# GrumpyZhou/patch2pix

Measured on AMD Instinct MI355X. Metric: image-pairs/sec (480x640, ptmax=400), matching hot path, feature pyramids resident in HBM, higher is better.
Workload: dtype f32-equivalent: fp16x2 (every f32 operand, scaled by an exact power of two, = sum of 2 fp16 planes to within 2^-24 of its magnitude; 3 fp16 MFMA products per f32 product, f32 accumulate); second convolution as Winograd F(2x2,3x3) (transforms in f32, filters transformed in f64)

## Files before the change

patch2pix_amd/csrc/regress_wino.hip:

```cpp
#ifndef WNPL
#define WNPL 2
#endif
#include "regress_common.h"

#include <algorithm>
#include <cmath>
#include <vector>

#undef WNS
#if WNPL == 1
#define WNS(f) fp16x1::f
#else
#define WNS(f) f
#endif

namespace p2p {
#if WNPL == 1
namespace fp16x1 {
#endif

typedef _Float16 we8 __attribute__((ext_vector_type(8)));
#define WMFMA(a, b, c) __builtin_amdgcn_mfma_f32_32x32x16_f16(__builtin_bit_cast(we8, (a)), __builtin_bit_cast(we8, (b)), (c), 0, 0, 0)

constexpr int WNT = 512;
constexpr int WBLK = WNPL * (WINO_BLK / 2);
constexpr int WPIECE = WBLK / 8;
constexpr int WSTAGE = 2 * WBLK;
constexpr int WRING = 4;
constexpr int WLDS = WRING * WSTAGE;
static_assert(WINO_BLK == 2 * 128 * 64, "block = [plane 2][row 128][32 K of fp16]");

struct WinoArgs {
    const unsigned char *U;
    const unsigned char *Wt;
    const float *bn2s, *bn2b;
    const float *hinv;
    float *V;
    int mblocks;
    int p0, n;
    const int *dev_counts;
    int nitems;
    int start[MAXB + 1];
};

#if WNPL == 2
#define WDMA(ga_, gb_, la_)                                                                                            \
        P2P_GLOBAL_LOAD_LDS16(ga_ + lane16, la_, 0); P2P_GLOBAL_LOAD_LDS16(ga_ + lane16, la_, 1024);                   \
        P2P_GLOBAL_LOAD_LDS16(gb_ + lane16, la_ + WBLK, 0); P2P_GLOBAL_LOAD_LDS16(gb_ + lane16, la_ + WBLK, 1024);
#define WWAIT_TWO_IN_FLIGHT() P2P_WAIT_VMCNT(8)
#define WWAIT_ONE_IN_FLIGHT() P2P_WAIT_VMCNT(4)
#else
#undef WDMA
#undef WWAIT_TWO_IN_FLIGHT
#undef WWAIT_ONE_IN_FLIGHT
#define WDMA(ga_, gb_, la_)                                                                                            \
        P2P_GLOBAL_LOAD_LDS16(ga_ + lane16, la_, 0); P2P_GLOBAL_LOAD_LDS16(gb_ + lane16, la_ + WBLK, 0);
#define WWAIT_TWO_IN_FLIGHT() P2P_WAIT_VMCNT(4)
#define WWAIT_ONE_IN_FLIGHT() P2P_WAIT_VMCNT(2)
#endif
#define WISSUE(ST, SLOT)                                                                                               \
    {                                                                                                                  \
        const int st_ = (ST) < 256 ? (ST) : 255;            \
        const int p_ = st_ >> 4, kc_ = st_ & 15;                                                                       \
        const unsigned char *ga_ = a.U + ((size_t)(p_ * a.mblocks + mb) * 16 + kc_) * WBLK + woff;                      \
        const unsigned char *gb_ = a.Wt + ((size_t)((p_ * 4 + nb) * 16 + kc_)) * WBLK + woff;                           \
        unsigned char *la_ = smb + (SLOT) * WSTAGE + wave * WPIECE;                                                    \
        WDMA(ga_, gb_, la_)                                                                                            \
    }
#define WREAD(FA, FB, SLOT, S)                                                                                         \
    {                                                                                                                  \
        const unsigned char *pa_ = smb + (SLOT) * WSTAGE + ((S) ? aoff1 : aoff0);                                      \
        const unsigned char *pb_ = smb + (SLOT) * WSTAGE + WBLK + ((S) ? boff1 : boff0);                                \
        _Pragma("unroll") for (int q_ = 0; q_ < WNPL; ++q_) {                                                           \
            FA[0][q_] = *(const f32x4 *)(pa_ + q_ * 8192);                                                             \
            FA[1][q_] = *(const f32x4 *)(pa_ + 2048 + q_ * 8192);                                                      \
            FB[q_] = *(const f32x4 *)(pb_ + q_ * 8192);                                                                \
        }                                                                                                              \
    }
#if WNPL == 2
#define WSLAB_(FA, FB, C0, C1)                                                                                         \
    M0 = WMFMA(FA[0][1], FB[0], C0); M1 = WMFMA(FA[1][1], FB[0], C1);                                                  \
    M0 = WMFMA(FA[0][0], FB[1], M0); M1 = WMFMA(FA[1][0], FB[1], M1);                                                  \
    M0 = WMFMA(FA[0][0], FB[0], M0); M1 = WMFMA(FA[1][0], FB[0], M1);
#else
#undef WSLAB_
#define WSLAB_(FA, FB, C0, C1) M0 = WMFMA(FA[0][0], FB[0], C0); M1 = WMFMA(FA[1][0], FB[0], C1);
#endif
#define WSLAB(FA, FB) WSLAB_(FA, FB, M0, M1)
#define WSLABZ(FA, FB) WSLAB_(FA, FB, zero16, zero16)

#if WNPL == 2
#define WPIPE_A()                                                                                                      \
    _Pragma("unroll") for (int g_ = 0; g_ < 6; ++g_) {                                                                 \
        __builtin_amdgcn_sched_group_barrier(0x008, 1, 0); __builtin_amdgcn_sched_group_barrier(0x100, 1, 0); }        \
    __builtin_amdgcn_sched_barrier(0);
#define WPIPE_B()                                                                                                      \
    _Pragma("unroll") for (int g_ = 0; g_ < 4; ++g_) {                                                                 \
        __builtin_amdgcn_sched_group_barrier(0x008, 1, 0); __builtin_amdgcn_sched_group_barrier(0x010, 1, 0);          \
        __builtin_amdgcn_sched_group_barrier(0x100, 1, 0); }                                                           \
    _Pragma("unroll") for (int g_ = 0; g_ < 2; ++g_) {                                                                 \
        __builtin_amdgcn_sched_group_barrier(0x008, 1, 0); __builtin_amdgcn_sched_group_barrier(0x100, 1, 0); }        \
    __builtin_amdgcn_sched_barrier(0);
#else
#undef WPIPE_A
#undef WPIPE_B
#define WPIPE_A()                                                                                                      \
    __builtin_amdgcn_sched_group_barrier(0x008, 1, 0); __builtin_amdgcn_sched_group_barrier(0x100, 2, 0);              \
    __builtin_amdgcn_sched_group_barrier(0x008, 1, 0); __builtin_amdgcn_sched_group_barrier(0x100, 1, 0);              \
    __builtin_amdgcn_sched_barrier(0);
#define WPIPE_B()                                                                                                      \
    __builtin_amdgcn_sched_group_barrier(0x008, 1, 0); __builtin_amdgcn_sched_group_barrier(0x010, 1, 0);              \
    __builtin_amdgcn_sched_group_barrier(0x100, 2, 0);                                                                 \
    __builtin_amdgcn_sched_group_barrier(0x008, 1, 0); __builtin_amdgcn_sched_group_barrier(0x010, 1, 0);              \
    __builtin_amdgcn_sched_group_barrier(0x100, 1, 0);                                                                 \
    __builtin_amdgcn_sched_barrier(0);
#endif

__global__ __launch_bounds__(WNT, 1) void wino_gemm_kernel(WinoArgs a) {
    P2P_DYN_SHARED(unsigned char, smb);
    const int tid = threadIdx.x;
    const int wave = __builtin_amdgcn_readfirstlane(tid >> 6);
    const int lane = tid & 63, l31 = lane & 31, half = lane >> 5;
    const int g = blockIdx.x, xcd = g & 7, q = g >> 3;
    const int nb = q & 3, mb = (q >> 2) * 8 + xcd;
    if (mb >= a.mblocks || wino_slot(a, a.p0 + mb * 8) < 0) return;
    const int wm = wave >> 2, wn = wave & 3;
    const unsigned lane16 = lane * 16, woff = wave * WPIECE;
    const int sw = (l31 >> 2) & 3;
    const unsigned aoff0 = ((wm * 64 + l31) * 4 + ((0 + half) ^ sw)) * 16, aoff1 = ((wm * 64 + l31) * 4 + ((2 + half) ^ sw)) * 16;
    const unsigned boff0 = ((wn * 32 + l31) * 4 + ((0 + half) ^ sw)) * 16, boff1 = ((wn * 32 + l31) * 4 + ((2 + half) ^ sw)) * 16;

    const f32x16 zero16 = {0};
    f32x16 Y[4][2];
#pragma unroll
    for (int ab = 0; ab < 4; ++ab)
#pragma unroll
        for (int t = 0; t < 2; ++t) Y[ab][t] = zero16;
    f32x4 XA[2][WNPL], XB[WNPL], YA[2][WNPL], YB[WNPL];

    WISSUE(0, 0) WISSUE(1, 1) WISSUE(2, 2)
    WWAIT_TWO_IN_FLIGHT();
    __builtin_amdgcn_s_barrier();
    WREAD(XA, XB, 0, 0)
    __builtin_amdgcn_sched_barrier(0);

#pragma unroll 1
    for (int p = 0; p < 16; ++p) {
        f32x16 M0, M1;
#pragma unroll
        for (int kc = 0; kc < 16; ++kc) {
            const int slot = kc & 3;
            WREAD(YA, YB, slot, 1)
            if (kc == 0) { WSLABZ(XA, XB) } else { WSLAB(XA, XB) }
            WPIPE_A()
            WWAIT_ONE_IN_FLIGHT();
            __builtin_amdgcn_s_barrier();
            __builtin_amdgcn_sched_barrier(0);
            WISSUE(p * 16 + kc + 3, (kc + 3) & 3)
            WREAD(XA, XB, (kc + 1) & 3, 0)
            WSLAB(YA, YB)
            WPIPE_B()
        }
        {
            const int i = p >> 2, j = p & 3;
            const float ca[2] = {(i < 3) ? 1.f : 0.f, (i == 0) ? 0.f : (i == 1) ? 1.f : -1.f};
            const float cb[2] = {(j < 3) ? 1.f : 0.f, (j == 0) ? 0.f : (j == 1) ? 1.f : -1.f};
#pragma unroll
            for (int ab = 0; ab < 4; ++ab) {
                const float c = ca[ab >> 1] * cb[ab & 1];
                Y[ab][0] += c * M0; Y[ab][1] += c * M1;
            }
        }
    }
    P2P_WAIT_VMCNT(0);

    const int n = nb * 128 + wn * 32 + l31;
    const float s = a.bn2s[n], b = a.bn2b[n];
#pragma unroll
    for (int t = 0; t < 2; ++t)
#pragma unroll
        for (int gq = 0; gq < 2; ++gq) {
            const int pl = mb * 8 + wm * 4 + 2 * t + gq;
            const int slot = wino_slot(a, a.p0 + pl);
            const float hs = s * a.hinv[pl];
            float m = 0.f;
#pragma unroll
            for (int ab = 0; ab < 4; ++ab)
#pragma unroll
                for (int r = 0; r < 8; ++r) m = fmaxf(m, fmaf(Y[ab][t][8 * gq + r], hs, b));
            m = fmaxf(m, __shfl_xor(m, 32));
            if (half == 0 && slot >= 0) a.V[(size_t)slot * 512 + n] = m;
        }
}

__global__ __launch_bounds__(WNT) void wino_zero_tail_kernel(WinoArgs a, unsigned char *U, float *hinv, int p1) {
    const int mb = blockIdx.x, tid = threadIdx.x, wave = tid >> 6, lane = tid & 63;
    if (wino_slot(a, a.p0 + mb * 8) < 0) return;
    for (int j = 1; j < 8; ++j) {
        const int c = a.p0 + mb * 8 + j;
        if (c < p1 && wino_slot(a, c) >= 0) continue;
        const unsigned rr = (unsigned)j * 16u + ((unsigned)lane >> 2);
        const unsigned inblk = (rr * 4u + (((unsigned)lane & 3u) ^ ((rr >> 2) & 3u))) * 16u;
        const size_t pstride = (size_t)a.mblocks * (16u * WBLK);
        for (int i2 = 0; i2 < 2; ++i2) {
            unsigned char *ub = U + (size_t)(((unsigned)mb * 16u + (unsigned)(wave * 2 + i2)) * (unsigned)WBLK + inblk);
            for (int pos = 0; pos < 16; ++pos) {
                *(uint4 *)(ub + pos * pstride) = make_uint4(0u, 0u, 0u, 0u);
#if WNPL == 2
                *(uint4 *)(ub + pos * pstride + WINO_BLK / 2) = make_uint4(0u, 0u, 0u, 0u);
#endif
            }
        }
        if (tid == 0) hinv[mb * 8 + j] = 0.f;
    }
}

#if WNPL == 2
__global__ __launch_bounds__(NT, 2) void regress_fc_kernel(RegressArgs args, int lvl) {
    P2P_DYN_SHARED(unsigned char, smb);
    fc_batch_parse(args.reg[lvl], args, lvl, args.ws + (size_t)lvl * args.n * 512,
                   args.ws + ((2 * (size_t)args.n * 512 + 31) & ~(size_t)31), smb, threadIdx.x);
}
#endif

void pack_wino_weights(const float *conv2_w, float *out, int *t2) {
    static const double G[4][3] = {{1, 0, 0}, {0.5, 0.5, 0.5}, {0.5, -0.5, 0.5}, {0, 0, 1}};
    std::vector<double> wt((size_t)16 * 512 * 512);
    std::vector<double> mx(512, 0.0);
    for (int n = 0; n < 512; ++n)
        for (int k = 0; k < 512; ++k) {
            const float *gk = conv2_w + ((size_t)n * 512 + k) * 9;
            double tmp[4][3];
            for (int i = 0; i < 4; ++i)
                for (int b = 0; b < 3; ++b) tmp[i][b] = G[i][0] * gk[0 * 3 + b] + G[i][1] * gk[1 * 3 + b] + G[i][2] * gk[2 * 3 + b];
            for (int i = 0; i < 4; ++i)
                for (int j = 0; j < 4; ++j) {
                    const double v = tmp[i][0] * G[j][0] + tmp[i][1] * G[j][1] + tmp[i][2] * G[j][2];
                    wt[((size_t)(i * 4 + j) * 512 + n) * 512 + k] = v;
                    mx[n] = std::max(mx[n], std::fabs(v));
                }
        }
    for (int n = 0; n < 512; ++n) t2[n] = plane_exponent(mx[n]);
    uint16_t *d = (uint16_t *)out;
    for (int p = 0; p < 16; ++p)
        for (int n = 0; n < 512; ++n) {
            const int nb = n >> 7, col = n & 127;
            for (int k = 0; k < 512; ++k) {
                const int kc = k >> 5, qq = (k >> 3) & 3, e = k & 7;
                const float v = (float)std::ldexp(wt[((size_t)p * 512 + n) * 512 + k], t2[n]);
                const size_t blk = ((size_t)(p * 4 + nb) * 16 + kc) * (WBLK / 2);
                const size_t in = (size_t)(col * 4 + (qq ^ ((col >> 2) & 3))) * 8 + e;
#if WNPL == 2
                split_fp16_planes(v, &d[blk + in], &d[blk + 128 * 32 + in]);
#else
                d[blk + in] = round_fp16(v);
#endif
            }
        }
}

int launch_regress_wino(const RegressArgs &args, int n, hipStream_t stream) {
    RegressArgs a = args;
    static DeviceOnce attr_set;
    const int dev = raise_lds_limit(attr_set, {{(const void *)wino_gemm_kernel, (int)WLDS}, {(const void *)regress_fc_kernel, (int)FC_LDS_BYTES}});
    if (dev < 0) return dev;
    const int ncu = device_cu_count(dev);
    if (ncu < 0) return ncu;
    P2P_REQUIRE(a.ws, P2P_EINVAL, "%s: the scratch buffer is missing", "launch_regress_wino");
    unsigned char *wsU = (unsigned char *)(a.ws + wino_u_offset_floats((size_t)n));
    float *hinv = a.ws + wino_hinv_offset_floats((size_t)n);
    for (int lvl = 0; lvl < a.nlevels; ++lvl) {
        for (int ch = 0, nch = wino_nchunks((size_t)n); ch < nch; ++ch) {
            int p0, p1;
            wino_chunk_range((size_t)n, ch, &p0, &p1);
            const int cn = p1 - p0, mblocks = (cn + 7) / 8;
            if (cn <= 0) continue;
            a.lvl0 = lvl; a.p0 = p0; a.p1 = p0 + cn; a.wU = wsU; a.hinv = hinv; a.mblocks = mblocks;
            WinoArgs w;
            w.U = wsU; w.Wt = (const unsigned char *)a.reg[lvl].ww2; w.bn2s = a.reg[lvl].bn2s_w; w.bn2b = a.reg[lvl].bn2b;
            w.hinv = hinv; w.V = a.ws + (size_t)lvl * n * 512; w.mblocks = mblocks; w.p0 = p0; w.n = n;
            w.dev_counts = a.dev_counts; w.nitems = a.nitems;
            for (int b = 0; b <= MAXB; ++b) w.start[b] = a.start[b];
            int st = P2P_OK;
            if (a.dev_counts || (cn & 7)) {
                const int mb0 = a.dev_counts ? 0 : mblocks - 1;
                WinoArgs wz = w;
                wz.p0 = p0 + mb0 * 8;
                hipLaunchKernelGGL(wino_zero_tail_kernel, dim3(mblocks - mb0), dim3(WNT), 0, stream, wz,
                                   wsU + (size_t)mb0 * 16 * WBLK, hinv + mb0 * 8, p0 + cn);
                st = check_launch("wino_zero_tail_kernel");
                if (st != P2P_OK) return st;
            }
            st = WNS(launch_regress_h2_conv1)(a, cn, stream);
            if (st != P2P_OK) return st;
            hipLaunchKernelGGL(wino_gemm_kernel, dim3(((mblocks + 7) / 8) * 32), dim3(WNT), WLDS, stream, w);
            st = check_launch("wino_gemm_kernel");
            if (st != P2P_OK) return st;
        }
        hipLaunchKernelGGL(regress_fc_kernel, dim3(std::min(n, ncu)), dim3(NT), FC_LDS_BYTES, stream, a, lvl);
        const int st = check_launch("regress_fc_kernel");
        if (st != P2P_OK) return st;
    }
    return P2P_OK;
}

#if WNPL == 1
}
#endif
}

#if WNPL == 2
#undef WNPL
#define WNPL 1
#include "regress_wino.hip"
#endif
```

patch2pix_amd/ops.py:

```python
import ctypes
import math
import os

import numpy as np
import torch

from . import _lib, staging


def _stream():
    return ctypes.c_void_p(torch.cuda.current_stream().cuda_stream)


def _f32c(t, name):
    if t.dtype != torch.float32 or not t.is_cuda:
        raise TypeError(f"{name} must be a float32 tensor on the GPU (got {t.dtype}, {t.device})")
    return t.contiguous()


def _host(t):
    return t.detach().to("cpu", torch.float32).contiguous()


RELEASED_NCN_LAYOUT = dict(kernel_sizes=[3, 3], channels=[16, 1], symmetric_mode=True)
NCN_MAX_LAYERS, NCN_KERNEL_SIZES, NCN_MAX_CHANNELS = 4, (3, 5), 16


def ncn_layout(source=None, symmetric_mode=None):
    if source is None:
        lay = {k: (list(v) if isinstance(v, list) else v) for k, v in RELEASED_NCN_LAYOUT.items()}
    elif isinstance(source, dict) and any(str(k).startswith("conv.") for k in source):
        ks, ch, cin, i = [], [], 1, 0
        while f"conv.{2 * i}.weight" in source:
            shp = tuple(source[f"conv.{2 * i}.weight"].shape)
            if len(shp) != 6 or len({shp[0], shp[3], shp[4], shp[5]}) != 1:
                raise ValueError(f"conv.{2 * i}.weight has shape {shp}: expected the stored layout [k, c_out, c_in, k, k, k]")
            if shp[2] != cin:
                raise ValueError(f"conv.{2 * i}.weight has {shp[2]} input channels where the layer below it gives {cin}")
            bias = source.get(f"conv.{2 * i}.bias")
            if bias is None or tuple(bias.shape) != (shp[1],):
                raise ValueError(f"conv.{2 * i}.bias is missing or is not of shape ({shp[1]},)")
            ks.append(int(shp[0])); ch.append(int(shp[1])); cin = shp[1]; i += 1
        if not ks:
            raise ValueError("no conv.0.weight among the consensus tensors")
        lay = dict(kernel_sizes=ks, channels=ch, symmetric_mode=True)
    else:
        get = (lambda k, d=None: source.get(k, d)) if isinstance(source, dict) else (lambda k, d=None: getattr(source, k, d))
        ks, ch = get("kernel_sizes"), get("channels")
        if ks is None or ch is None:
            raise ValueError("a consensus configuration needs kernel_sizes and channels")
        lay = dict(kernel_sizes=[int(k) for k in ks], channels=[int(c) for c in ch], symmetric_mode=bool(get("symmetric_mode", True)))
    if symmetric_mode is not None:
        lay["symmetric_mode"] = bool(symmetric_mode)
    ks, ch = lay["kernel_sizes"], lay["channels"]
    if not ks or len(ks) != len(ch):
        raise ValueError(f"kernel_sizes {ks} and channels {ch} must be non-empty lists of one length")
    if any(k <= 0 for k in ks) or any(c <= 0 for c in ch):
        raise ValueError(f"kernel_sizes {ks} / channels {ch}: sizes must be positive")
    if len(ks) > NCN_MAX_LAYERS:
        raise NotImplementedError(f"kernel_sizes {ks}: at most {NCN_MAX_LAYERS} consensus layers are implemented")
    if any(k not in NCN_KERNEL_SIZES for k in ks):
        raise NotImplementedError(f"kernel_sizes {ks}: kernel sizes 3 and 5 are implemented")
    if any(c > NCN_MAX_CHANNELS for c in ch):
        raise NotImplementedError(f"channels {ch}: at most {NCN_MAX_CHANNELS} channels per layer are implemented")
    if ch[-1] != 1:
        raise NotImplementedError(f"channels {ch}: the last layer must have one channel (the volume is [B,1,...] downstream)")
    return lay


def ncn_shapes(lay):
    shapes, cin = {}, 1
    for i, (k, c) in enumerate(zip(lay["kernel_sizes"], lay["channels"])):
        shapes[f"conv.{2 * i}.weight"], shapes[f"conv.{2 * i}.bias"] = (k, c, cin, k, k, k), (c,)
        cin = c
    return shapes


def coarse_mode_id(mode):
    if not isinstance(mode, str) or mode not in _lib.COARSE_MODES:
        raise ValueError(f"unknown coarse mode {mode!r}: one of {sorted(_lib.COARSE_MODES)}")
    return _lib.COARSE_MODES[mode]


def default_coarse_mode():
    return os.environ.get("P2P_COARSE_MODE") or "fp16x2"


class NcnWeights:

    layout, generic = RELEASED_NCN_LAYOUT, False

    def __init__(self, w1, b1, w2, b2, device):
        keep = [_host(w1), _host(b1), _host(w2), _host(b2)]
        if tuple(keep[0].shape) != (3, 16, 1, 3, 3, 3) or tuple(keep[2].shape) != (3, 1, 16, 3, 3, 3):
            raise NotImplementedError("only NeighConsensus(kernel_sizes=[3,3], channels=[16,1]) is implemented")
        self.handle = ctypes.c_void_p()
        with torch.cuda.device(device):
            _lib.check(_lib.p2p_ncn_create(*[t.data_ptr() for t in keep], ctypes.byref(self.handle)), "p2p_ncn_create")
        self.device = torch.device(device)
        if default_coarse_mode() != "fp16x2":
            self.set_mode(default_coarse_mode())

    @classmethod
    def from_state_dict(cls, sd, device, symmetric_mode=True, generic=False):
        lay = ncn_layout({k: v for k, v in sd.items() if k.startswith("conv.")}, symmetric_mode)
        if not generic and lay == RELEASED_NCN_LAYOUT:
            return cls(sd["conv.0.weight"], sd["conv.0.bias"], sd["conv.2.weight"], sd["conv.2.bias"], device)
        n = len(lay["kernel_sizes"])
        keep = [(_host(sd[f"conv.{2 * i}.weight"]), _host(sd[f"conv.{2 * i}.bias"])) for i in range(n)]
        c, t = _lib.NcnConfig(), _lib.NcnTensors()
        c.n_layers, c.symmetric = n, int(lay["symmetric_mode"])
        for i in range(n):
            c.kernel_size[i], c.channels[i] = lay["kernel_sizes"][i], lay["channels"][i]
            t.w[i], t.b[i] = keep[i][0].data_ptr(), keep[i][1].data_ptr()
        self = cls.__new__(cls)
        self.handle = ctypes.c_void_p()
        with torch.cuda.device(device):
            _lib.check(_lib.p2p_ncn_create_config(ctypes.byref(c), ctypes.byref(t), ctypes.byref(self.handle)), "p2p_ncn_create_config")
        self.device, self.layout, self.generic = torch.device(device), lay, True
        return self

    def set_tile(self, ta=0, tb=0, tc=0):
        if self.generic:
            raise NotImplementedError("set_tile: a generic consensus handle has no work-group tile to force")
        _lib.check(_lib.p2p_ncn_set_tile(self.handle, int(ta), int(tb), int(tc)), "p2p_ncn_set_tile")

    def set_mode(self, mode):
        mid = coarse_mode_id(mode)
        if self.generic:
            raise NotImplementedError("set_mode: a generic consensus handle runs exact fp32 kernels and has no modes")
        _lib.check(_lib.p2p_ncn_set_mode(self.handle, mid), "p2p_ncn_set_mode")

    @property
    def mode(self):
        mid = _lib.p2p_ncn_get_mode(self.handle)
        return next(k for k, v in _lib.COARSE_MODES.items() if v == mid)

    def __del__(self):
        if getattr(self, "handle", None) and _lib is not None:
            _lib.p2p_ncn_destroy(self.handle)
            self.handle = None


def _parse_conv_tile(text):
    try:
        t = tuple(int(v) for v in text.split(","))
    except ValueError:
        t = ()
    if len(t) != 3 or min(t) < 0:
        raise ValueError(f"P2P_CONV_TILE={text!r}: expected three non-negative integers 'mt,nt,wn'")
    return t


FORCED_CONV_TILE = _parse_conv_tile(os.environ["P2P_CONV_TILE"]) if os.environ.get("P2P_CONV_TILE") else None


def backbone_mode_id(mode):
    if mode not in _lib.BACKBONE_MODES:
        raise ValueError(f"unknown backbone mode {mode!r}: one of {sorted(_lib.BACKBONE_MODES)}")
    return _lib.BACKBONE_MODES[mode]


def default_backbone_mode():
    return os.environ.get("P2P_BACKBONE_MODE") or "fp16x2"


class _BackboneMode:

    def set_mode(self, mode):
        _lib.check(self._set_mode(self.handle, backbone_mode_id(mode)), self._set_mode.__name__)

    @property
    def mode(self):
        mid = self._get_mode(self.handle)
        return next(k for k, v in _lib.BACKBONE_MODES.items() if v == mid)


class ConvBN(_BackboneMode):
    _set_mode, _get_mode = staticmethod(_lib.p2p_conv_set_mode), staticmethod(_lib.p2p_conv_get_mode)

    def __init__(self, conv_weight, bn_weight, bn_bias, bn_mean, bn_var, stride, device):
        keep = [_host(t) for t in (conv_weight, bn_weight, bn_bias, bn_mean, bn_var)]
        co, ci, ks, ks2 = keep[0].shape
        if ks != ks2:
            raise NotImplementedError("square kernels only")
        bn = _lib.BnParams(*[t.data_ptr() for t in keep[1:]])
        self.handle = ctypes.c_void_p()
        with torch.cuda.device(device):
            _lib.check(_lib.p2p_conv_create(keep[0].data_ptr(), ctypes.byref(bn), ci, co, ks, int(stride), ctypes.byref(self.handle)),
                       "p2p_conv_create")
        self.ci, self.co, self.ks, self.stride = ci, co, ks, int(stride)
        self.device = torch.device(device)
        self._tile = None
        if default_backbone_mode() != "fp16x2":
            self.set_mode(default_backbone_mode())

    def __del__(self):
        if getattr(self, "handle", None) and _lib is not None:
            _lib.p2p_conv_destroy(self.handle)
            self.handle = None

    def forward(self, x, xmax, residual=None, relu=True, ymax=None):
        n, h, w, ci = x.shape
        if ci != self.ci or x.dtype != torch.float32 or not x.is_cuda or not x.is_contiguous():
            raise TypeError(f"ConvBN.forward: expected a contiguous float32 NHWC tensor with {self.ci} channels on the GPU")
        if FORCED_CONV_TILE != self._tile:
            _lib.check(_lib.p2p_conv_set_tile(self.handle, *(FORCED_CONV_TILE or (0, 0, 0))), "p2p_conv_set_tile")
            self._tile = FORCED_CONV_TILE
        pad = self.ks // 2
        ho, wo = (h + 2 * pad - self.ks) // self.stride + 1, (w + 2 * pad - self.ks) // self.stride + 1
        y = torch.empty((n, ho, wo, self.co), device=x.device, dtype=torch.float32)
        if residual is not None and (residual.shape != y.shape or not residual.is_contiguous()):
            raise TypeError("ConvBN.forward: residual must be a contiguous NHWC tensor of the output's shape")
        _lib.check(_lib.p2p_conv_forward(self.handle, x.data_ptr(), xmax.data_ptr(), n, h, w,
                                         residual.data_ptr() if residual is not None else None, int(relu), y.data_ptr(),
                                         ymax.data_ptr() if ymax is not None else None, _stream()), "p2p_conv_forward")
        return y


class Stem(_BackboneMode):
    _set_mode, _get_mode = staticmethod(_lib.p2p_stem_set_mode), staticmethod(_lib.p2p_stem_get_mode)

    def __init__(self, conv_weight, bn_weight, bn_bias, bn_mean, bn_var, device):
        keep = [_host(t) for t in (conv_weight, bn_weight, bn_bias, bn_mean, bn_var)]
        if tuple(keep[0].shape) != (64, 3, 7, 7):
            raise NotImplementedError("only the ResNet stem Conv2d(3, 64, 7, 2, 3) is implemented")
        bn = _lib.BnParams(*[t.data_ptr() for t in keep[1:]])
        self.handle = ctypes.c_void_p()
        with torch.cuda.device(device):
            _lib.check(_lib.p2p_stem_create(keep[0].data_ptr(), ctypes.byref(bn), ctypes.byref(self.handle)), "p2p_stem_create")
        self.device = torch.device(device)
        if default_backbone_mode() != "fp16x2":
            self.set_mode(default_backbone_mode())

    def __del__(self):
        if getattr(self, "handle", None) and _lib is not None:
            _lib.p2p_stem_destroy(self.handle)
            self.handle = None

    def forward(self, image):
        image = _f32c(image, "image")
        n, c, h, w = image.shape
        if c != 3:
            raise TypeError("Stem.forward: three-channel images only")
        imax = absmax_batch(image)
        y = torch.empty((n, 64, (h - 1) // 2 + 1, (w - 1) // 2 + 1), device=image.device, dtype=torch.float32)
        _lib.check(_lib.p2p_stem_forward(self.handle, image.data_ptr(), imax.data_ptr(), n, h, w, y.data_ptr(), _stream()), "p2p_stem_forward")
        return y


def maxpool_nhwc(x, ymax=None):
    x = _f32c(x, "x")
    n, c, h, w = x.shape
    y = torch.empty((n, (h - 1) // 2 + 1, (w - 1) // 2 + 1, c), device=x.device, dtype=torch.float32)
    _lib.check(_lib.p2p_maxpool_nhwc(x.data_ptr(), n, c, h, w, y.data_ptr(), ymax.data_ptr() if ymax is not None else None, _stream()),
               "p2p_maxpool_nhwc")
    return y


def nhwc_to_nchw(x):
    x = _f32c(x, "x")
    n, h, w, c = x.shape
    y = torch.empty((n, c, h, w), device=x.device, dtype=torch.float32)
    _lib.check(_lib.p2p_nhwc_to_nchw(x.data_ptr(), n, h, w, c, y.data_ptr(), _stream()), "p2p_nhwc_to_nchw")
    return y


def absmax_batch(x):
    x = _f32c(x, "x")
    out = torch.empty((x.shape[0],), device=x.device, dtype=torch.int32)
    _lib.check(_lib.p2p_absmax_batch(x.data_ptr(), x[0].numel(), x.shape[0], out.data_ptr(), _stream()), "p2p_absmax_batch")
    return out


FEAT_DIMS = (3, 64, 64, 128, 256)
RELEASED_LAYOUT = dict(feat_idx=[0, 1, 2, 3], feat_comb="pre", conv_dims=[512, 512], conv_kers=[3, 3], conv_strs=[2, 1],
                       fc_dims=[512, 256], psize=[16, 16])


def regressor_layout(config=None, feat_idx=None):
    get = (lambda k, d=None: config.get(k, d)) if isinstance(config, dict) else (lambda k, d=None: getattr(config, k, d))
    lay = {k: (list(v) if isinstance(v, list) else v) for k, v in RELEASED_LAYOUT.items()}
    if feat_idx is not None:
        lay["feat_idx"] = [int(i) for i in feat_idx]
    if config is not None:
        lay["feat_comb"] = get("feat_comb", "pre")
        lay["conv_dims"] = [int(d) for d in get("conv_dims")]
        lay["conv_kers"] = [int(k) for k in get("conv_kers")]
        strs = get("conv_strs")
        lay["conv_strs"] = [int(v) for v in strs] if strs is not None else [2] * len(lay["conv_kers"])
        lay["fc_dims"] = [int(d) for d in get("fc_dims")]
        ps = get("psize", [16, 16])
        lay["psize"] = [int(v) for v in ps] if isinstance(ps, (list, tuple)) else [int(ps), int(ps)]
    fi = lay["feat_idx"]
    if not fi or any(b <= a for a, b in zip(fi, fi[1:])) or any(i < 0 or i > 4 for i in fi):
        raise ValueError(f"feat_idx {fi}: a non-empty, strictly ascending list of pyramid levels")
    if 4 in fi:
        raise NotImplementedError(f"feat_idx {fi}: level 4 is not implemented by the fine stage (the pyramid handed to the "
                                  "library carries levels 0..3)")
    if lay["psize"] != [16, 16]:
        raise NotImplementedError(f"psize {lay['psize']}: psize must be [16,16]")
    if lay["feat_comb"] not in ("pre", "post"):
        raise ValueError(f"feat_comb {lay['feat_comb']!r}: 'pre' or 'post'")
    nc = len(lay["conv_dims"])
    if nc == 0 or len(lay["conv_kers"]) != nc or len(lay["conv_strs"]) != nc:
        raise ValueError("conv_dims, conv_kers and conv_strs must be non-empty lists of one length")
    if nc > 4 or len(lay["fc_dims"]) > 4:
        raise NotImplementedError("at most 4 convolutions and 4 hidden FC layers are implemented")
    for what in ("conv_dims", "fc_dims"):
        for d in lay[what]:
            if d <= 0:
                raise ValueError(f"{what} {lay[what]}: dims must be positive")
            if d % 16 or d > 1024:
                raise NotImplementedError(f"{what} {lay[what]}: dims must be multiples of 16 in [16, 1024]")
    side = 16
    for k, st in zip(lay["conv_kers"], lay["conv_strs"]):
        if k not in (1, 3, 5):
            raise NotImplementedError(f"conv_kers {lay['conv_kers']}: kernel sizes 1, 3 and 5 are implemented")
        if st not in (1, 2):
            raise NotImplementedError(f"conv_strs {lay['conv_strs']}: strides 1 and 2 are implemented")
        if side + 2 - k < 0:
            raise ValueError(f"conv_kers {lay['conv_kers']} / conv_strs {lay['conv_strs']}: the map shrinks below 1x1")
        side = (side + 2 - k) // st + 1
    return lay


def regressor_shapes(lay):
    feat_dim = sum(FEAT_DIMS[i] for i in lay["feat_idx"])
    cin = feat_dim if lay["feat_comb"] == "post" else 2 * feat_dim
    shapes, bns = {}, {}
    for i, (d, k) in enumerate(zip(lay["conv_dims"], lay["conv_kers"])):
        shapes[f"conv.{2 * i}.weight"] = (d, cin, k, k)
        bns[f"conv.{2 * i + 1}"] = d
        cin = d
    k = lay["conv_dims"][-1] * (2 if lay["feat_comb"] == "post" else 1)
    for i, d in enumerate(lay["fc_dims"]):
        shapes[f"fc.{3 * i}.weight"], shapes[f"fc.{3 * i}.bias"] = (d, k), (d,)
        bns[f"fc.{3 * i + 1}"] = d
        k = d
    n = 3 * len(lay["fc_dims"])
    shapes[f"fc.{n}.weight"], shapes[f"fc.{n}.bias"] = (5, k), (5,)
    return shapes, bns


class RegressorWeights:

    def __init__(self, sd, device, config=None, feat_idx=None, generic=False):
        lay = regressor_layout(config, feat_idx)
        self.layout = lay
        self.generic = bool(generic) or lay != RELEASED_LAYOUT
        self.device = torch.device(device)
        if self.generic:
            self._create_generic(sd, lay)
            return
        exp = {"conv.0.weight": (512, 518, 3, 3), "conv.2.weight": (512, 512, 3, 3), "fc.0.weight": (512, 512),
               "fc.3.weight": (256, 512), "fc.6.weight": (5, 256)}
        for k, shp in exp.items():
            if tuple(sd[k].shape) != shp:
                raise NotImplementedError(f"regressor {k} has shape {tuple(sd[k].shape)}; only the released "
                                          f"configuration {shp} is implemented")
        keep = {k: _host(v) for k, v in sd.items() if v.is_floating_point()}
        p = _lib.RegressorParams()

        def bn(prefix):
            return _lib.BnParams(keep[prefix + ".weight"].data_ptr(), keep[prefix + ".bias"].data_ptr(),
                                 keep[prefix + ".running_mean"].data_ptr(), keep[prefix + ".running_var"].data_ptr())

        p.conv1_w = keep["conv.0.weight"].data_ptr(); p.bn1 = bn("conv.1")
        p.conv2_w = keep["conv.2.weight"].data_ptr(); p.bn2 = bn("conv.3")
        p.fc1_w = keep["fc.0.weight"].data_ptr(); p.fc1_b = keep["fc.0.bias"].data_ptr(); p.bnf1 = bn("fc.1")
        p.fc2_w = keep["fc.3.weight"].data_ptr(); p.fc2_b = keep["fc.3.bias"].data_ptr(); p.bnf2 = bn("fc.4")
        p.fc3_w = keep["fc.6.weight"].data_ptr(); p.fc3_b = keep["fc.6.bias"].data_ptr()
        self.handle = ctypes.c_void_p()
        with torch.cuda.device(device):
            _lib.check(_lib.p2p_regressor_create(ctypes.byref(p), ctypes.byref(self.handle)), "p2p_regressor_create")
        env = os.environ.get("P2P_REGRESS_MODE")
        if env:
            self.set_mode(env)

    def _create_generic(self, sd, lay):
        shapes, bns = regressor_shapes(lay)
        for k, shp in shapes.items():
            if k not in sd or tuple(sd[k].shape) != shp:
                got = tuple(sd[k].shape) if k in sd else "no tensor"
                raise ValueError(f"regressor {k}: the configuration asks for shape {shp}, the state_dict has {got}")
        keep = {k: _host(v) for k, v in sd.items() if v.is_floating_point()}

        def bn(prefix):
            return _lib.BnParams(keep[prefix + ".weight"].data_ptr(), keep[prefix + ".bias"].data_ptr(),
                                 keep[prefix + ".running_mean"].data_ptr(), keep[prefix + ".running_var"].data_ptr())

        c, t = _lib.RegressorConfig(), _lib.RegressorTensors()
        c.n_feat = len(lay["feat_idx"])
        for i, j in enumerate(lay["feat_idx"]):
            c.feat_idx[i] = j
        c.feat_comb = _lib.FEAT_COMB[lay["feat_comb"]]
        c.n_conv, c.n_fc, c.psize = len(lay["conv_dims"]), len(lay["fc_dims"]), lay["psize"][0]
        for i in range(c.n_conv):
            c.conv_dim[i], c.conv_ker[i], c.conv_str[i] = lay["conv_dims"][i], lay["conv_kers"][i], lay["conv_strs"][i]
            t.conv_w[i] = keep[f"conv.{2 * i}.weight"].data_ptr()
            t.conv_bn[i] = bn(f"conv.{2 * i + 1}")
        for i in range(c.n_fc):
            c.fc_dim[i] = lay["fc_dims"][i]
            t.fc_w[i], t.fc_b[i] = keep[f"fc.{3 * i}.weight"].data_ptr(), keep[f"fc.{3 * i}.bias"].data_ptr()
            t.fc_bn[i] = bn(f"fc.{3 * i + 1}")
        t.out_w, t.out_b = keep[f"fc.{3 * c.n_fc}.weight"].data_ptr(), keep[f"fc.{3 * c.n_fc}.bias"].data_ptr()
        self.handle = ctypes.c_void_p()
        with torch.cuda.device(self.device):
            _lib.check(_lib.p2p_regressor_create_config(ctypes.byref(c), ctypes.byref(t), ctypes.byref(self.handle)),
                       "p2p_regressor_create_config")

    def set_mode(self, mode):
        if self.generic:
            if mode == "generic":
                return
            raise NotImplementedError(f"regressor mode {mode!r}: a generic regressor runs the exact-fp32 generic kernels only")
        modes = {**_lib.REGRESS_MODES, **_lib.REGRESS_MODES_LOSSY}
        if mode not in modes:
            removed = {"bf16x2": "round 5", "bf16x3": "round 4"}
            why = f" ({mode!r} was removed in {removed[mode]})" if mode in removed else ""
            raise ValueError(f"unknown regressor mode {mode!r}{why}: one of {sorted(modes)}")
        with torch.cuda.device(self.device):
            _lib.check(_lib.p2p_regressor_set_mode(self.handle, modes[mode]), "p2p_regressor_set_mode")

    @property
    def mode(self):
        code = _lib.p2p_regressor_get_mode(self.handle)
        names = {v: k for k, v in {**_lib.REGRESS_MODES, **_lib.REGRESS_MODES_LOSSY}.items()}
        return "generic" if code == _lib.REGRESS_GENERIC else names[code]

    def __del__(self):
        if getattr(self, "handle", None) and _lib is not None:
            _lib.p2p_regressor_destroy(self.handle)
            self.handle = None


_workspaces = {}

regress_events = None


def _workspace(device, nbytes):
    key = (device.index, torch.cuda.current_stream(device).cuda_stream)
    ws = _workspaces.get(key)
    if ws is None or ws.numel() < nbytes:
        ws = torch.empty(nbytes, dtype=torch.uint8, device=device)
        _workspaces[key] = ws
    return ws


COARSE_WORKSPACE_LIMIT = 16 << 30


def coarse_forward_batch(feat_a, feat_b, ksize, ncn, want_delta=True, out_corr=None, out_delta=None):
    feat_a, feat_b = _f32c(feat_a, "feat_a"), _f32c(feat_b, "feat_b")
    if feat_a.dim() != 4 or feat_b.dim() != 4 or feat_a.shape[0] != feat_b.shape[0]:
        raise ValueError("coarse_forward_batch expects [B,C,h,w] feature maps with equal B")
# ... 511 lines not shown
```

Before: 959.7.

## Split tail Winograd GEMM blocks into half-M tiles to balance the last wave

Adds a templated half-height (64-row) variant of the Winograd GEMM tile and launches the trailing M blocks as two half tiles each, chosen so the work fills the CUs more evenly when 4*mblocks does not divide the CU count. The goal is less idle time from a partial last wave of workgroups. Half tiles reload the full B operand per half, so there is more load traffic and a lower MFMA-to-load ratio on those blocks. A runtime split mode (default 1) is exposed through an environment variable.

```diff
diff --git a/patch2pix_amd/csrc/regress_wino.hip b/patch2pix_amd/csrc/regress_wino.hip
--- a/patch2pix_amd/csrc/regress_wino.hip
+++ b/patch2pix_amd/csrc/regress_wino.hip
@@ -38,6 +38,7 @@
     float *V;
     int mblocks;
     int p0, n;
+    int mbfull;
     const int *dev_counts;
     int nitems;
     int start[MAXB + 1];
@@ -47,25 +48,35 @@
 #define WDMA(ga_, gb_, la_)                                                                                            \
         P2P_GLOBAL_LOAD_LDS16(ga_ + lane16, la_, 0); P2P_GLOBAL_LOAD_LDS16(ga_ + lane16, la_, 1024);                   \
         P2P_GLOBAL_LOAD_LDS16(gb_ + lane16, la_ + WBLK, 0); P2P_GLOBAL_LOAD_LDS16(gb_ + lane16, la_ + WBLK, 1024);
-#define WWAIT_TWO_IN_FLIGHT() P2P_WAIT_VMCNT(8)
-#define WWAIT_ONE_IN_FLIGHT() P2P_WAIT_VMCNT(4)
 #else
 #undef WDMA
-#undef WWAIT_TWO_IN_FLIGHT
-#undef WWAIT_ONE_IN_FLIGHT
+#undef WDMA_HALF
 #define WDMA(ga_, gb_, la_)                                                                                            \
         P2P_GLOBAL_LOAD_LDS16(ga_ + lane16, la_, 0); P2P_GLOBAL_LOAD_LDS16(gb_ + lane16, la_ + WBLK, 0);
-#define WWAIT_TWO_IN_FLIGHT() P2P_WAIT_VMCNT(4)
-#define WWAIT_ONE_IN_FLIGHT() P2P_WAIT_VMCNT(2)
-#endif
+#endif
+#if WNPL == 2
+#define WDMA_HALF(ga_, gb_, la_, lb_)                                                                                  \
+        P2P_GLOBAL_LOAD_LDS16(ga_ + lane16, la_, 0);                                                                   \
+        P2P_GLOBAL_LOAD_LDS16(gb_ + lane16, lb_, 0); P2P_GLOBAL_LOAD_LDS16(gb_ + lane16, lb_, 1024);
+#else
+#define WDMA_HALF(ga_, gb_, la_, lb_)                                                                                  \
+        P2P_GLOBAL_LOAD_LDS16(ga_ + lane16, la_, 0); P2P_GLOBAL_LOAD_LDS16(gb_ + lane16, lb_, 0);
+#endif
+#define WWAIT_TWO_IN_FLIGHT() wino_wait_vmcnt<2 * (MT == 2 ? 2 * WNPL : WNPL + 1)>()
+#define WWAIT_ONE_IN_FLIGHT() wino_wait_vmcnt<(MT == 2 ? 2 * WNPL : WNPL + 1)>()
 #define WISSUE(ST, SLOT)                                                                                               \
     {                                                                                                                  \
         const int st_ = (ST) < 256 ? (ST) : 255;            \
         const int p_ = st_ >> 4, kc_ = st_ & 15;                                                                       \
-        const unsigned char *ga_ = a.U + ((size_t)(p_ * a.mblocks + mb) * 16 + kc_) * WBLK + woff;                      \
         const unsigned char *gb_ = a.Wt + ((size_t)((p_ * 4 + nb) * 16 + kc_)) * WBLK + woff;                           \
-        unsigned char *la_ = smb + (SLOT) * WSTAGE + wave * WPIECE;                                                    \
-        WDMA(ga_, gb_, la_)                                                                                            \
+        if constexpr (MT == 2) {                                                                                       \
+            const unsigned char *ga_ = a.U + ((size_t)(p_ * a.mblocks + mb) * 16 + kc_) * WBLK + woff;                  \
+            unsigned char *la_ = smb + (SLOT) * WSTAGE + wave * WPIECE;                                                \
+            WDMA(ga_, gb_, la_)                                                                                        \
+        } else {                                                                                                       \
+            const unsigned char *ga_ = a.U + ((size_t)(p_ * a.mblocks + mb) * 16 + kc_) * WBLK + hoff;                  \
+            WDMA_HALF(ga_, gb_, smb + (SLOT) * WSTAGE + hoff, smb + (SLOT) * WSTAGE + WBLK + woff)                      \
+        }                                                                                                              \
     }
 #define WREAD(FA, FB, SLOT, S)                                                                                         \
     {                                                                                                                  \
@@ -73,18 +84,24 @@
         const unsigned char *pb_ = smb + (SLOT) * WSTAGE + WBLK + ((S) ? boff1 : boff0);                                \
         _Pragma("unroll") for (int q_ = 0; q_ < WNPL; ++q_) {                                                           \
             FA[0][q_] = *(const f32x4 *)(pa_ + q_ * 8192);                                                             \
-            FA[1][q_] = *(const f32x4 *)(pa_ + 2048 + q_ * 8192);                                                      \
+            if constexpr (MT == 2) FA[1][q_] = *(const f32x4 *)(pa_ + 2048 + q_ * 8192);                               \
             FB[q_] = *(const f32x4 *)(pb_ + q_ * 8192);                                                                \
         }                                                                                                              \
     }
 #if WNPL == 2
 #define WSLAB_(FA, FB, C0, C1)                                                                                         \
-    M0 = WMFMA(FA[0][1], FB[0], C0); M1 = WMFMA(FA[1][1], FB[0], C1);                                                  \
-    M0 = WMFMA(FA[0][0], FB[1], M0); M1 = WMFMA(FA[1][0], FB[1], M1);                                                  \
-    M0 = WMFMA(FA[0][0], FB[0], M0); M1 = WMFMA(FA[1][0], FB[0], M1);
+    if constexpr (MT == 2) {                                                                                           \
+        M0 = WMFMA(FA[0][1], FB[0], C0); M1 = WMFMA(FA[1][1], FB[0], C1);                                              \
+        M0 = WMFMA(FA[0][0], FB[1], M0); M1 = WMFMA(FA[1][0], FB[1], M1);                                              \
+        M0 = WMFMA(FA[0][0], FB[0], M0); M1 = WMFMA(FA[1][0], FB[0], M1);                                              \
+    } else {                                                                                                           \
+        M0 = WMFMA(FA[0][1], FB[0], C0); M0 = WMFMA(FA[0][0], FB[1], M0); M0 = WMFMA(FA[0][0], FB[0], M0);             \
+    }
 #else
 #undef WSLAB_
-#define WSLAB_(FA, FB, C0, C1) M0 = WMFMA(FA[0][0], FB[0], C0); M1 = WMFMA(FA[1][0], FB[0], C1);
+#define WSLAB_(FA, FB, C0, C1)                                                                                         \
+    M0 = WMFMA(FA[0][0], FB[0], C0);                                                                                   \
+    if constexpr (MT == 2) M1 = WMFMA(FA[1][0], FB[0], C1);
 #endif
 #define WSLAB(FA, FB) WSLAB_(FA, FB, M0, M1)
 #define WSLABZ(FA, FB) WSLAB_(FA, FB, zero16, zero16)
@@ -115,28 +132,63 @@
     __builtin_amdgcn_sched_group_barrier(0x100, 1, 0);                                                                 \
     __builtin_amdgcn_sched_barrier(0);
 #endif
-
-__global__ __launch_bounds__(WNT, 1) void wino_gemm_kernel(WinoArgs a) {
-    P2P_DYN_SHARED(unsigned char, smb);
+#if WNPL == 2
+#define WPIPE_A_HALF()                                                                                                 \
+    __builtin_amdgcn_sched_group_barrier(0x008, 1, 0); __builtin_amdgcn_sched_group_barrier(0x100, 2, 0);              \
+    _Pragma("unroll") for (int g_ = 0; g_ < 2; ++g_) {                                                                 \
+        __builtin_amdgcn_sched_group_barrier(0x008, 1, 0); __builtin_amdgcn_sched_group_barrier(0x100, 1, 0); }        \
+    __builtin_amdgcn_sched_barrier(0);
+#define WPIPE_B_HALF()                                                                                                 \
+    __builtin_amdgcn_sched_group_barrier(0x008, 1, 0); __builtin_amdgcn_sched_group_barrier(0x010, 1, 0);              \
+    __builtin_amdgcn_sched_group_barrier(0x100, 2, 0);                                                                 \
+    _Pragma("unroll") for (int g_ = 0; g_ < 2; ++g_) {                                                                 \
+        __builtin_amdgcn_sched_group_barrier(0x008, 1, 0); __builtin_amdgcn_sched_group_barrier(0x010, 1, 0);          \
+        __builtin_amdgcn_sched_group_barrier(0x100, 1, 0); }                                                           \
+    __builtin_amdgcn_sched_barrier(0);
+#else
+#undef WPIPE_A_HALF
+#undef WPIPE_B_HALF
+#define WPIPE_A_HALF()                                                                                                 \
+    __builtin_amdgcn_sched_group_barrier(0x008, 1, 0); __builtin_amdgcn_sched_group_barrier(0x100, 2, 0);              \
+    __builtin_amdgcn_sched_barrier(0);
+#define WPIPE_B_HALF()                                                                                                 \
+    __builtin_amdgcn_sched_group_barrier(0x008, 1, 0); __builtin_amdgcn_sched_group_barrier(0x010, 2, 0);              \
+    __builtin_amdgcn_sched_group_barrier(0x100, 2, 0);                                                                 \
+    __builtin_amdgcn_sched_barrier(0);
+#endif
+
+#if WNPL == 2
+template <int N>
+__device__ __forceinline__ void wino_wait_vmcnt() {
+    static_assert(N == 2 || N == 3 || N == 4 || N == 6 || N == 8, "pieces in flight: one or two stages of 2, 3 or 4 pieces per wave");
+    if constexpr (N == 2) P2P_WAIT_VMCNT(2);
+    if constexpr (N == 3) P2P_WAIT_VMCNT(3);
+    if constexpr (N == 4) P2P_WAIT_VMCNT(4);
+    if constexpr (N == 6) P2P_WAIT_VMCNT(6);
+    if constexpr (N == 8) P2P_WAIT_VMCNT(8);
+}
+#endif
+
+template <int MT>
+__device__ __forceinline__ void wino_gemm_tile(const WinoArgs &a, unsigned char *smb, const int mb, const int nb, const int h) {
     const int tid = threadIdx.x;
     const int wave = __builtin_amdgcn_readfirstlane(tid >> 6);
     const int lane = tid & 63, l31 = lane & 31, half = lane >> 5;
-    const int g = blockIdx.x, xcd = g & 7, q = g >> 3;
-    const int nb = q & 3, mb = (q >> 2) * 8 + xcd;
-    if (mb >= a.mblocks || wino_slot(a, a.p0 + mb * 8) < 0) return;
     const int wm = wave >> 2, wn = wave & 3;
     const unsigned lane16 = lane * 16, woff = wave * WPIECE;
+    [[maybe_unused]] const unsigned hoff = ((wave >> 2) & (WNPL - 1)) * 8192 + h * 4096 + (wave & 3) * 1024;
     const int sw = (l31 >> 2) & 3;
-    const unsigned aoff0 = ((wm * 64 + l31) * 4 + ((0 + half) ^ sw)) * 16, aoff1 = ((wm * 64 + l31) * 4 + ((2 + half) ^ sw)) * 16;
+    const int arow = (MT == 2 ? wm * 64 : h * 64 + wm * 32) + l31;
+    const unsigned aoff0 = (arow * 4 + ((0 + half) ^ sw)) * 16, aoff1 = (arow * 4 + ((2 + half) ^ sw)) * 16;
     const unsigned boff0 = ((wn * 32 + l31) * 4 + ((0 + half) ^ sw)) * 16, boff1 = ((wn * 32 + l31) * 4 + ((2 + half) ^ sw)) * 16;
 
     const f32x16 zero16 = {0};
-    f32x16 Y[4][2];
+    f32x16 Y[4][MT];
 #pragma unroll
     for (int ab = 0; ab < 4; ++ab)
 #pragma unroll
-        for (int t = 0; t < 2; ++t) Y[ab][t] = zero16;
-    f32x4 XA[2][WNPL], XB[WNPL], YA[2][WNPL], YB[WNPL];
+        for (int t = 0; t < MT; ++t) Y[ab][t] = zero16;
+    f32x4 XA[MT][WNPL], XB[WNPL], YA[MT][WNPL], YB[WNPL];
 
     WISSUE(0, 0) WISSUE(1, 1) WISSUE(2, 2)
     WWAIT_TWO_IN_FLIGHT();
@@ -146,20 +198,21 @@
 
 #pragma unroll 1
     for (int p = 0; p < 16; ++p) {
-        f32x16 M0, M1;
+        f32x16 M0;
+        [[maybe_unused]] f32x16 M1;
 #pragma unroll
         for (int kc = 0; kc < 16; ++kc) {
             const int slot = kc & 3;
             WREAD(YA, YB, slot, 1)
             if (kc == 0) { WSLABZ(XA, XB) } else { WSLAB(XA, XB) }
-            WPIPE_A()
+            if constexpr (MT == 2) { WPIPE_A() } else { WPIPE_A_HALF() }
             WWAIT_ONE_IN_FLIGHT();
             __builtin_amdgcn_s_barrier();
             __builtin_amdgcn_sched_barrier(0);
             WISSUE(p * 16 + kc + 3, (kc + 3) & 3)
             WREAD(XA, XB, (kc + 1) & 3, 0)
             WSLAB(YA, YB)
-            WPIPE_B()
+            if constexpr (MT == 2) { WPIPE_B() } else { WPIPE_B_HALF() }
         }
         {
             const int i = p >> 2, j = p & 3;
@@ -168,7 +221,8 @@
 #pragma unroll
             for (int ab = 0; ab < 4; ++ab) {
                 const float c = ca[ab >> 1] * cb[ab & 1];
-                Y[ab][0] += c * M0; Y[ab][1] += c * M1;
+                Y[ab][0] += c * M0;
+                if constexpr (MT == 2) Y[ab][1] += c * M1;
             }
         }
     }
@@ -177,10 +231,10 @@
     const int n = nb * 128 + wn * 32 + l31;
     const float s = a.bn2s[n], b = a.bn2b[n];
 #pragma unroll
-    for (int t = 0; t < 2; ++t)
+    for (int t = 0; t < MT; ++t)
 #pragma unroll
         for (int gq = 0; gq < 2; ++gq) {
-            const int pl = mb * 8 + wm * 4 + 2 * t + gq;
+            const int pl = mb * 8 + (MT == 2 ? wm * 4 + 2 * t : h * 4 + wm * 2) + gq;
             const int slot = wino_slot(a, a.p0 + pl);
             const float hs = s * a.hinv[pl];
             float m = 0.f;
@@ -191,6 +245,23 @@
             m = fmaxf(m, __shfl_xor(m, 32));
             if (half == 0 && slot >= 0) a.V[(size_t)slot * 512 + n] = m;
         }
+}
+
+__global__ __launch_bounds__(WNT, 1) void wino_gemm_kernel(WinoArgs a) {
+    P2P_DYN_SHARED(unsigned char, smb);
+    const int g = blockIdx.x, xcd = g & 7, gfull = ((a.mbfull + 7) >> 3) * 32;
+    if (g < gfull) {
+        const int q = g >> 3;
+        const int nb = q & 3, mb = (q >> 2) * 8 + xcd;
+        if (mb >= a.mbfull || wino_slot(a, a.p0 + mb * 8) < 0) return;
+        wino_gemm_tile<2>(a, smb, mb, nb, 0);
+    } else {
+        const int q = (g - gfull) >> 3;
+        const int nb = q & 3, hb = (q >> 2) * 8 + xcd;
+        const int mb = a.mbfull + (hb >> 1), h = hb & 1;
+        if (mb >= a.mblocks || wino_slot(a, a.p0 + mb * 8 + h * 4) < 0) return;
+        wino_gemm_tile<1>(a, smb, mb, nb, h);
+    }
 }
 
 __global__ __launch_bounds__(WNT) void wino_zero_tail_kernel(WinoArgs a, unsigned char *U, float *hinv, int p1) {
@@ -257,6 +328,29 @@
 #endif
             }
         }
+}
+
+#if WNPL == 2
+static std::atomic<int> g_wino_split{1};
+int wino_split_mode(int set) {
+    if (set >= 0 && set <= 2) g_wino_split.store(set, std::memory_order_relaxed);
+    return g_wino_split.load(std::memory_order_relaxed);
+}
+
+int wino_full_blocks(int mblocks, int ncu, int split) {
+    if (split == 2) return 0;
+    const int rem = (4 * mblocks) % ncu;
+    if (split == 0 || rem == 0 || rem > ncu / 2) return mblocks;
+    return mblocks - (rem + 3) / 4;
+}
+#endif
+
+int launch_wino_gemm(const WinoArgs &args, int ncu, hipStream_t stream) {
+    WinoArgs w = args;
+    w.mbfull = wino_full_blocks(w.mblocks, ncu, wino_split_mode(-1));
+    const int grid = ((w.mbfull + 7) / 8) * 32 + ((2 * (w.mblocks - w.mbfull) + 7) / 8) * 32;
+    hipLaunchKernelGGL(wino_gemm_kernel, dim3(grid), dim3(WNT), WLDS, stream, w);
+    return check_launch("wino_gemm_kernel");
 }
 
 int launch_regress_wino(const RegressArgs &args, int n, hipStream_t stream) {
@@ -278,7 +372,7 @@
             a.lvl0 = lvl; a.p0 = p0; a.p1 = p0 + cn; a.wU = wsU; a.hinv = hinv; a.mblocks = mblocks;
             WinoArgs w;
             w.U = wsU; w.Wt = (const unsigned char *)a.reg[lvl].ww2; w.bn2s = a.reg[lvl].bn2s_w; w.bn2b = a.reg[lvl].bn2b;
-            w.hinv = hinv; w.V = a.ws + (size_t)lvl * n * 512; w.mblocks = mblocks; w.p0 = p0; w.n = n;
+            w.hinv = hinv; w.V = a.ws + (size_t)lvl * n * 512; w.mblocks = mblocks; w.mbfull = mblocks; w.p0 = p0; w.n = n;
             w.dev_counts = a.dev_counts; w.nitems = a.nitems;
             for (int b = 0; b <= MAXB; ++b) w.start[b] = a.start[b];
             int st = P2P_OK;
@@ -293,8 +387,7 @@
             }
             st = WNS(launch_regress_h2_conv1)(a, cn, stream);
             if (st != P2P_OK) return st;
-            hipLaunchKernelGGL(wino_gemm_kernel, dim3(((mblocks + 7) / 8) * 32), dim3(WNT), WLDS, stream, w);
-            st = check_launch("wino_gemm_kernel");
+            st = WNS(launch_wino_gemm)(w, ncu, stream);
             if (st != P2P_OK) return st;
         }
         hipLaunchKernelGGL(regress_fc_kernel, dim3(std::min(n, ncu)), dim3(NT), FC_LDS_BYTES, stream, a, lvl);
diff --git a/patch2pix_amd/ops.py b/patch2pix_amd/ops.py
--- a/patch2pix_amd/ops.py
+++ b/patch2pix_amd/ops.py
@@ -153,6 +153,20 @@
 
 
 FORCED_CONV_TILE = _parse_conv_tile(os.environ["P2P_CONV_TILE"]) if os.environ.get("P2P_CONV_TILE") else None
+
+
+def set_wino_split(mode):
+    mode = int(mode)
+    if mode not in (0, 1, 2):
+        raise ValueError(f"P2P_WINO_SPLIT={mode!r}: expected 0, 1 or 2")
+    fn = getattr(_lib.lib, "_ZN3p2p15wino_split_modeEi")
+    fn.restype, fn.argtypes = ctypes.c_int, [ctypes.c_int]
+    assert fn(mode) == mode
+    return mode
+
+
+if os.environ.get("P2P_WINO_SPLIT"):
+    set_wino_split(os.environ["P2P_WINO_SPLIT"])
 
 
 def backbone_mode_id(mode):
```

Result: no change. 960.3 (median of 3 runs) (+0.1%).
